# soham2560/MPCHoloNavigation

Measured on AMD Instinct MI355X. Metric: rollouts/sec per computeVelocityCommands() tick, higher is better.
Workload: dtype f32

## Files before the change

mpcholonavigation_amd/csrc/smpc_api.cpp:

```cpp

#include "smpc_ctx.h"

#include <emmintrin.h>

namespace smpc_impl {

thread_local std::string g_create_error;

int fail(smpc_ctx* c, int code, const std::string& msg)
{
  if (c) c->err = msg; else g_create_error = msg;
  return code;
}

int wait_map_upload(smpc_ctx* c)
{
  if (!c->map_pending) return SMPC_OK;
  HIPCK(c, hipEventSynchronize(c->ev_map));
  c->map_pending = false;
  return SMPC_OK;
}

void bar_copy(void* dev_dst, const void* host_src, size_t n)
{
// ... 495 lines not shown
  if (cfg->motion_model > SMPC_MODEL_ACKERMANN)
    return fail(nullptr, SMPC_ERR_UNSUPPORTED, "motion_model must be Omni, DiffDrive or Ackermann");
  if (cfg->motion_model == SMPC_MODEL_ACKERMANN && !(cfg->ackermann_min_turning_r >= 0.f))
    return fail(nullptr, SMPC_ERR_INVALID, "ackermann_min_turning_r must be >= 0");
  if (cfg->time_steps > 64 * SMPC_MAX_R)
    return fail(nullptr, SMPC_ERR_UNSUPPORTED, "time_steps > 256");
  if (!(cfg->temperature > 0.f) || !(cfg->model_dt > 0.f))
    return fail(nullptr, SMPC_ERR_INVALID, "temperature and model_dt must be > 0");
  int ndev = 0;
  hipError_t e = hipGetDeviceCount(&ndev);
  if (e != hipSuccess || ndev == 0)
    return fail(nullptr, SMPC_ERR_DEVICE,
                std::string("no HIP device: ") + (e != hipSuccess ? hipGetErrorString(e) : "count 0") +
                " (libsmpc has no CPU fallback)");
  smpc_ctx* c = new (std::nothrow) smpc_ctx();
  if (!c) return fail(nullptr, SMPC_ERR_NOMEM, "out of host memory");
  c->cfg = *cfg;
  c->knobs = read_knobs();
  smpc_critic_params_default(&c->critics);
  c->holonomic = cfg->motion_model == SMPC_MODEL_OMNI;
  c->acker_r = cfg->motion_model == SMPC_MODEL_ACKERMANN ? cfg->ackermann_min_turning_r : -1.f;
  c->c_vx_max = cfg->vx_max; c->c_vx_min = cfg->vx_min; c->c_vy = cfg->vy_max; c->c_wz = cfg->wz_max;
  int dev = cfg->device;
  if (dev < 0) {
    if (hipGetDevice(&dev) != hipSuccess) dev = 0;
  }
  c->device = dev;
#define CK(call)                                                                        \
  do {                                                                                  \
    hipError_t e__ = (call);                                                            \
    if (e__ != hipSuccess) {                                                            \
      g_create_error = std::string(#call) + ": " + hipGetErrorString(e__);              \
      free_ctx(c);                                                                      \
      return SMPC_ERR_DEVICE;                                                           \
    }                                                                                   \
  } while (0)
  CK(hipSetDevice(dev));
  hipDeviceProp_t prop;
  CK(hipGetDeviceProperties(&prop, dev));
  c->num_cu = prop.multiProcessorCount > 0 ? prop.multiProcessorCount : 256;
  {
    int large_bar = 0;
    if (hipDeviceGetAttribute(&large_bar, hipDeviceAttributeIsLargeBar, dev) != hipSuccess) large_bar = 0;
    c->bar_tick = large_bar != 0 && c->knobs.bar_tick;
    if (c->bar_tick && c->knobs.hdp_flush) {
      c->hdp_flush = find_hdp_flush(dev);
      if (!c->hdp_flush) c->bar_tick = false;
    }
  }
  CK(hipStreamCreateWithFlags(&c->own_stream, hipStreamNonBlocking));
  c->stream = c->own_stream;
  if (getenv("SMPC_LANE_TIMELINE")) {
    static_assert(SMPC_TAIL_STAMPS_AT == 8192 + kMaxGrid * 8, "the tail's stamps sit behind the lane pass's");
    CK(hipMalloc(&c->d_timeline, (8192 + kMaxGrid * 8 + 8 * 16) * sizeof(unsigned long long)));
    CK(hipMemset(c->d_timeline, 0, (8192 + kMaxGrid * 8 + 8 * 16) * sizeof(unsigned long long)));
  }
  CK(hipEventCreate(&c->ev0));
  CK(hipEventCreateWithFlags(&c->ev_map, hipEventDisableTiming));
  CK(hipEventCreate(&c->ev1));
  for (auto& e : c->evp) CK(hipEventCreate(&e));
  const uint32_t T = cfg->time_steps;
  c->R = T <= 64 ? 1 : (T <= 128 ? 2 : 4);
  const size_t n = static_cast<size_t>(cfg->batch_size) * T * sizeof(float);
  CK(hipMalloc(&c->d_nvx, n));
  CK(hipMalloc(&c->d_nvy, n));
  if (!c->holonomic) CK(hipMemset(c->d_nvy, 0, n));
  CK(hipMalloc(&c->d_nwz, n));
  {
    bool tpr = cfg->batch_size >= kLaneMinBatch && cfg->time_steps <= kLaneMaxT;
    if (cfg->time_steps <= 64 && cfg->time_steps >= 36 && (cfg->time_steps & 3u) == 0 && cfg->batch_size >= kSplitMinBatch &&
        !c->knobs.no_split)
      tpr = true;
    if (cfg->flags & SMPC_FLAG_WAVE_PER_ROLLOUT) tpr = false;
    if (cfg->flags & SMPC_FLAG_LANE_PER_ROLLOUT) {
      tpr = true;
      c->lane_forced = true;
    }
    if (c->knobs.pass == Knobs::kWave) tpr = false;
    if (c->knobs.pass == Knobs::kLane || c->knobs.pass == Knobs::kSplit) {
      tpr = true;
      c->lane_forced = true;
    }
    if (cfg->flags & SMPC_FLAG_STORE_TRAJECTORIES) tpr = false;
    const size_t ngm = static_cast<size_t>(SMPC_GM_ROLLOUTS(cfg->batch_size)) * T * sizeof(float);
    if (3ull * ngm >= (1ull << 32)) tpr = false;
    c->use_tpr = tpr;
    if (tpr) {
      CK(hipMalloc(&c->d_tvx, 3 * ngm));
      c->d_tvy = c->d_tvx + ngm / sizeof(float);
      c->d_twz = c->d_tvy + ngm / sizeof(float);
      if (!c->holonomic) CK(hipMemset(c->d_tvy, 0, ngm));
      CK(lane_set_lds_limit(static_cast<int>(kLdsPerCu)));
      CK(split_set_lds_limit(static_cast<int>(kLdsPerCu)));
    }
  }
  CK(hipMalloc(&c->d_costs[0], cfg->batch_size * sizeof(float)));
  CK(hipMalloc(&c->d_costs[1], cfg->batch_size * sizeof(float)));
  CK(hipMemset(c->d_costs[0], 0, cfg->batch_size * sizeof(float)));
  CK(hipMemset(c->d_costs[1], 0, cfg->batch_size * sizeof(float)));
  if (cfg->flags & SMPC_FLAG_STORE_TRAJECTORIES) {
    for (int i = 0; i < 3; ++i) {
      CK(hipMalloc(&c->d_traj[i], n));
      CK(hipMemset(c->d_traj[i], 0, n));
    }
  }
  c->tick_cap = tick_layout(T, SMPC_MAX_PATH).total;
  CK(hipMalloc(&c->d_tick, c->tick_cap));
  CK(hipHostMalloc(&c->h_tick, c->tick_cap, hipHostMallocDefault));
// ... 526 lines not shown
  return SMPC_OK;
}

int smpc_set_stream(smpc_ctx* c, void* hip_stream)
{
  if (!c) return SMPC_ERR_INVALID;
  const int rc = wait_map_upload(c);
  if (rc != SMPC_OK) return rc;
  c->stream = hip_stream == SMPC_STREAM_OWN ? c->own_stream : static_cast<hipStream_t>(hip_stream);
  return SMPC_OK;
}

int smpc_debug_tail_timeline(smpc_ctx* c, unsigned long long* out)
{
  if (!c || !out || !c->d_timeline) return SMPC_ERR_INVALID;
  HIPCK(c, hipSetDevice(c->device));
  HIPCK(c, hipStreamSynchronize(c->stream));
  HIPCK(c, hipMemcpy(out, c->d_timeline + SMPC_TAIL_STAMPS_AT, 8 * 16 * sizeof(unsigned long long), hipMemcpyDeviceToHost));
  return SMPC_OK;
}

int smpc_debug_lane_timeline(smpc_ctx* c, double* out, uint32_t* n_blocks)
{
  if (!c || !out || !c->d_timeline) return SMPC_ERR_INVALID;
  HIPCK(c, hipSetDevice(c->device));
  HIPCK(c, hipStreamSynchronize(c->stream));
  const uint32_t nb = c->plan.lane.grid;
  std::vector<unsigned long long> h(static_cast<size_t>(nb) * 8);
  HIPCK(c, hipMemcpy(h.data(), c->d_timeline, h.size() * sizeof(h[0]), hipMemcpyDeviceToHost));
  unsigned long long t0 = ~0ull;
  for (uint32_t b = 0; b < nb; ++b) t0 = std::min(t0, h[b * 8]);
  for (int k = 0; k < 7; ++k) {
    std::vector<double> v;
    for (uint32_t b = 0; b < nb; ++b)
      if (h[b * 8 + k]) v.push_back(static_cast<double>(h[b * 8 + k] - (k ? h[b * 8 + k - 1] : t0)));
    std::sort(v.begin(), v.end());
    out[3 * k] = v.empty() ? 0 : v.front();
    out[3 * k + 1] = v.empty() ? 0 : v[v.size() / 2];
    out[3 * k + 2] = v.empty() ? 0 : v.back();
  }
  std::vector<unsigned long long> hw(static_cast<size_t>(nb) * 8);
  HIPCK(c, hipMemcpy(hw.data(), c->d_timeline + 8192, hw.size() * sizeof(hw[0]), hipMemcpyDeviceToHost));
  for (int w = 0; w < 8; ++w) {
    std::vector<double> v;
    for (uint32_t b = 0; b < nb; ++b)
      if (hw[b * 8 + w] && h[b * 8 + 2]) v.push_back(static_cast<double>(hw[b * 8 + w] - h[b * 8 + 2]));
    std::sort(v.begin(), v.end());
    out[21 + w] = v.empty() ? 0 : v[v.size() / 2];
  }
  if (n_blocks) *n_blocks = nb;
  return SMPC_OK;
}

const char* smpc_debug_last_pass_kernel(void) {return smpc_last_pass_kernel;}

int smpc_debug_bar_tick(const smpc_ctx* c) {return c && c->bar_tick ? 1 : 0;}

int smpc_set_profile(smpc_ctx* c, int enable)
{
  if (!c) return SMPC_ERR_INVALID;
  if (enable) c->cfg.flags |= SMPC_FLAG_PROFILE;
  else c->cfg.flags &= ~static_cast<uint32_t>(SMPC_FLAG_PROFILE);
  return SMPC_OK;
}
}
```

mpcholonavigation_amd/csrc/smpc_dev.h:

```cpp
#ifndef SMPC_DEV_H_
#define SMPC_DEV_H_

#include <stdint.h>

#define SD_OBSTACLES 0x001u
#define SD_PATH_ALIGN 0x002u
#define SD_PATH_FOLLOW 0x004u
#define SD_GOAL_ANGLE 0x008u
#define SD_PREFER_FORWARD 0x010u
#define SD_USE_PATH_YAW 0x020u
#define SD_ACCUMULATE 0x040u
#define SD_STORE_TRAJ 0x080u
#define SD_TRACK_UNKNOWN 0x100u
#define SD_NEED_FURTHEST 0x200u
#define SD_LOCAL_FURTHEST 0x400u
#define SD_CONSTRAINT 0x800u
#define SD_COST 0x1000u
#define SD_GOAL 0x2000u
#define SD_TWIRLING 0x4000u
#define SD_PATH_ANGLE 0x8000u
#define SD_DEADBAND 0x10000u
#define SD_FP_OBSTACLES 0x20000u
#define SD_FP_COST 0x40000u
#define SD_PATH_ALIGN_LEGACY 0x80000u
// ... 74 lines not shown
  float ga_weight, ga_goal_yaw;
  uint32_t ga_power;
  float pfw_weight;
  uint32_t pfw_power;
  float con_weight, con_max_vel, con_min_vel;
  uint32_t con_power;
  float con_acker_r;
  const float* lut_cost;
  float cost_w254, cost_collision_cost;
  float cost_critical;
  uint32_t cost_near_goal;
  uint32_t cost_power;
  double goal_x, goal_y;
  float goal_weight;
  uint32_t goal_power;
  float tw_weight;
  uint32_t tw_power;
  const uint8_t* pang_active;
  float pang_weight;
  uint32_t pang_power, pang_offset;
  int32_t pang_correct;
  const uint8_t* pal_active;
  float pal_weight, pal_eval;
  uint32_t pal_power;
  double db_vx, db_vy, db_wz;
  float db_weight;
  uint32_t db_power;
  uint32_t fp_n;
  float fp_pic;
  const SmpcLut* lut_fp;
  double fp_x[16], fp_y[16];
  float g_vx, g_vy, g_wz;
  float neg_inv_temp;
  float k2;
  float* partials;
  uint32_t* furthest_out;
  uint32_t tail;
  uint32_t* tail_counter;
  float* tuple;
  SmpcFinal fin;
  unsigned long long* timeline;
  uint32_t canary_echo;
  uint32_t tick_inline;
  uint32_t u_inline;
  uint16_t io_px, io_py, io_pyaw, io_D, io_pf_idx, io_pvalid, io_pa_active, io_pang_active, io_pal_active, io_pad;
  uint8_t tick_bytes[1536] __attribute__((aligned(16)));
  float u_arg[3 * 64] __attribute__((aligned(16)));
};
#define SMPC_INLINE_TICK_CAP 1536u
#define SMPC_MAX_GRID 2048u
#define SMPC_CANARY_SLOT(T) (SMPC_MAX_GRID * (4u + 3u * (T)))
#define SMPC_TAIL_MAX_GRID 512u
#define SMPC_TAIL_STAMPS_AT (8192u + 2048u * 8u)
static inline uint32_t smpc_tail_lds_bytes(uint32_t T) {return (512u + 64u + ((4u + 3u * T + 63u) / 64u) * 2048u + 4u) * 4u;}

#if defined(__HIPCC__)
struct SmpcTickPtrs {
  const float* u;
  const float* px;
  const float* py;
  const float* pyaw;
  const float* D;
  const uint32_t* pf_idx;
  const uint8_t* pvalid;
  const uint8_t* pa_active;
  const uint8_t* pang_active;
  const uint8_t* pal_active;
};
__device__ __forceinline__ SmpcTickPtrs smpc_tick_ptrs(const SmpcDev& p, bool kernarg_is_dev)
{
  SmpcTickPtrs t{p.u, p.px, p.py, p.pyaw, p.D, p.pf_idx, p.pvalid, p.pa_active, p.pang_active, p.pal_active};
#if defined(__HIP_DEVICE_COMPILE__)
  if (kernarg_is_dev && p.tick_inline) {
    const uint8_t* k = reinterpret_cast<const uint8_t*>(__builtin_amdgcn_kernarg_segment_ptr()) +
                       __builtin_offsetof(SmpcDev, tick_bytes);
    if (p.u_inline) t.u = reinterpret_cast<const float*>(reinterpret_cast<const uint8_t*>(__builtin_amdgcn_kernarg_segment_ptr()) +
                                                         __builtin_offsetof(SmpcDev, u_arg));
    t.px = reinterpret_cast<const float*>(k + p.io_px);
    t.py = reinterpret_cast<const float*>(k + p.io_py);
    t.pyaw = reinterpret_cast<const float*>(k + p.io_pyaw);
    t.D = reinterpret_cast<const float*>(k + p.io_D);
    t.pf_idx = reinterpret_cast<const uint32_t*>(k + p.io_pf_idx);
    t.pvalid = k + p.io_pvalid;
    t.pa_active = k + p.io_pa_active;
    t.pang_active = k + p.io_pang_active;
    t.pal_active = k + p.io_pal_active;
  }
#else
  (void)kernarg_is_dev;
#endif
  return t;
}
#endif

#if defined(__HIPCC__)
__host__ __device__
#endif
static inline uint32_t smpc_furthest_index(float F) {return (uint32_t)(F + 0.5f);}


#define SMPC_P2P_MAX_RANKS 16
struct SmpcP2P {
  float* peer[SMPC_P2P_MAX_RANKS];
  uint32_t world, rank;
  uint32_t slot_floats;
  uint32_t xseq;
// ... 28 lines not shown
```

mpcholonavigation_amd/csrc/smpc_lane.hip:

```cpp

#include <hip/hip_runtime.h>
#include <stdint.h>
#include <stdio.h>

#include <type_traits>

#include "smpc_dev.h"
#include "smpc_device_math.h"
#include "smpc_tail.h"
#include "smpc_lane_common.h"
#include "smpc_inst.h"

#ifndef WAVE
#define WAVE 64
#endif
#ifndef LANE_X_RR_NOLOAD
#define LANE_X_RR_NOLOAD 0
#endif
#define LANE_BLOCK 512
#ifndef LANE_BLOCK_RR
#define LANE_BLOCK_RR 512
#endif

#ifndef LANE_X_GAMMA_N
#define LANE_X_GAMMA_N 0
#endif
#ifndef LANE_X_GAMMA_UC
#define LANE_X_GAMMA_UC 1
#endif
#ifndef LANE_X_FURTHEST_WINDOW
#define LANE_X_FURTHEST_WINDOW 1
#endif
#ifndef LANE_X_PFW_MIN
#define LANE_X_PFW_MIN 1
#endif
#ifndef LANE_X_CELL_AX
#define LANE_X_CELL_AX 1
#endif
#ifndef LANE_X_PIN_LDS
#define LANE_X_PIN_LDS 0
#endif
#ifndef LANE_X_PARK_STEP
#define LANE_X_PARK_STEP 0
#endif
#ifndef LANE_X_CONST_VGPR
#define LANE_X_CONST_VGPR 0
#endif

#ifndef LANE_X_PFW_BARE
#define LANE_X_PFW_BARE 1
#endif
#ifndef LANE_X_NOISE_QUAD
#define LANE_X_NOISE_QUAD 1
#endif
#ifndef LANE_X_PRIO_ITER
#define LANE_X_PRIO_ITER 1
#endif

template <bool TO_GM>
__global__ void __launch_bounds__(256) smpc_relayout(const float* __restrict__ src, float* __restrict__ dst,
                                                    uint32_t B, uint32_t T)
{
  __shared__ float tile[32][33];
  const uint32_t b0 = blockIdx.x * 32, t0 = blockIdx.y * 32;
  const uint32_t lx = threadIdx.x & 31, ly = threadIdx.x >> 5;
  if (TO_GM) {
    for (uint32_t k = ly; k < 32; k += 8) {
      const uint32_t b = b0 + k, t = t0 + lx;
      tile[k][lx] = (b < B && t < T) ? src[(size_t)b * T + t] : 0.f;
    }
    __syncthreads();
    for (uint32_t k = ly; k < 32; k += 8) {
      const uint32_t t = t0 + k, b = b0 + lx;
      if (b < B && t < T) dst[SMPC_GM_INDEX(b, t, T)] = tile[lx][k];
    }
  } else {
    for (uint32_t k = ly; k < 32; k += 8) {
      const uint32_t t = t0 + k, b = b0 + lx;
      tile[lx][k] = (b < B && t < T) ? src[SMPC_GM_INDEX(b, t, T)] : 0.f;
    }
    __syncthreads();
    for (uint32_t k = ly; k < 32; k += 8) {
      const uint32_t b = b0 + k, t = t0 + lx;
      if (b < B && t < T) dst[(size_t)b * T + t] = tile[k][lx];
    }
  }
}

hipError_t smpc_launch_relayout(const float* src, float* dst, uint32_t B, uint32_t T, bool to_gm, hipStream_t st)
{
  const dim3 grid((B + 31) / 32, (T + 31) / 32);
  if (to_gm) hipLaunchKernelGGL(smpc_relayout<true>, grid, dim3(256), 0, st, src, dst, B, T);
  else hipLaunchKernelGGL(smpc_relayout<false>, grid, dim3(256), 0, st, src, dst, B, T);
  return hipGetLastError();
}

__global__ void __launch_bounds__(64) smpc_lane_reduce_kernel(const float* __restrict__ v,
                                                              const float* __restrict__ w,
                                                              float* __restrict__ out)
{
  const int lane = threadIdx.x;
  float V[64];
#pragma unroll
  for (int t = 0; t < 64; ++t) V[t] = v[lane * 64 + t];
  const LaneW lw = lane_weights(w[lane], lane);
  out[lane] = lane_reduce64(V, lw, lane);
}

hipError_t smpc_launch_lane_reduce(const float* v, const float* w, float* out, hipStream_t st)
// ... 114 lines not shown
```

mpcholonavigation_amd/csrc/smpc_lane_common.h:

```cpp
#ifndef SMPC_LANE_COMMON_H_
#define SMPC_LANE_COMMON_H_

#include <hip/hip_runtime.h>
#include <stdint.h>

#include "smpc_dev.h"
#include "smpc_device_math.h"

#ifndef WAVE
#define WAVE 64
#endif

typedef unsigned u32x2 __attribute__((ext_vector_type(2)));
typedef const float __attribute__((address_space(4))) * cfloat_p;
typedef float f32x32 __attribute__((ext_vector_type(32)));
typedef float f32x4 __attribute__((ext_vector_type(4)));
typedef float f32x2 __attribute__((ext_vector_type(2)));
#define LANE_PARK_STRIDE 68

struct LaneW {
  float wa, wb;
};

#define SMPC_DPP_NODE(NAME, CTRL, BANKS)                                                    \
// ... 13 lines not shown
template <int CTRL>
__device__ __forceinline__ float dpp_mov(float v)
{
  return __uint_as_float(
    (uint32_t)__builtin_amdgcn_update_dpp(0, (int)__float_as_uint(v), CTRL, 0xF, 0xF, false));
}

template <int K, int Rr>
__device__ __forceinline__ float lane_reduce_node(const float (&V)[64], const LaneW& w, int lane)
{
  if constexpr (K == 0) {
    return V[Rr];
  } else {
    const float a = lane_reduce_node<K - 1, Rr>(V, w, lane);
    const float b = lane_reduce_node<K - 1, Rr + (64 >> K)>(V, w, lane);
    if constexpr (K == 1) {
      const u32x2 s = __builtin_amdgcn_permlane32_swap(__float_as_uint(a), __float_as_uint(b),
                                                       false, false);
      return fmaf(w.wa, __uint_as_float(s.x), w.wb * __uint_as_float(s.y));
    } else if constexpr (K == 2) {
      const u32x2 s = __builtin_amdgcn_permlane16_swap(__float_as_uint(a), __float_as_uint(b),
                                                       false, false);
      return __uint_as_float(s.x) + __uint_as_float(s.y);
    } else if constexpr (K == 3) {
      return node_bit3(a, b);
    } else if constexpr (K == 4) {
      return node_bit2(a, b);
    } else if constexpr (K == 5) {
      const float ta = a + dpp_mov<0x4E>(a);
      const float tb = b + dpp_mov<0x4E>(b);
      return (lane & 2) ? tb : ta;
    } else {
      const float ta = a + dpp_mov<0xB1>(a);
      const float tb = b + dpp_mov<0xB1>(b);
      return (lane & 1) ? tb : ta;
    }
  }
}

__device__ __forceinline__ LaneW lane_weights(float w, int lane)
{
  const float wo = __shfl_xor(w, 32, WAVE);
  LaneW r;
  r.wa = lane < 32 ? w : wo;
  r.wb = lane < 32 ? wo : w;
  return r;
}

__device__ __forceinline__ float lane_reduce64(const float (&V)[64], const LaneW& w, int lane)
{
  return lane_reduce_node<6, 0>(V, w, lane);
}

__device__ __forceinline__ int cvt_floor_i32(float q)
{
  int r;
  asm("v_cvt_flr_i32_f32 %0, %1" : "=v"(r) : "v"(q));
  return r;
}

__device__ __forceinline__ float add_min_zero(float acc, float x)
{
  float m;
  asm("v_min_f32 %1, 0, %2\n\tv_add_f32 %0, %0, %1" : "+v"(acc), "=&v"(m) : "v"(x));
  return acc;
}

__device__ __forceinline__ uint32_t cell_byte_exact(const SmpcDev& p, uint8_t* s_map, float x,
                                                    float y, uint32_t slot)
{
  const uint32_t nwin = (uint32_t)(p.win_w * p.win_h);
  uint32_t mx = 0, my = 0;
  bool on = cell_index_exact((double)x, p.ox, p.res, p.W, mx);
  on = cell_index_exact((double)y, p.oy, p.res, p.H, my) && on;
  if (!on) return nwin;
  const uint32_t wx = mx - (uint32_t)p.win_x0, wy = my - (uint32_t)p.win_y0;
  if (wx < (uint32_t)p.win_w && wy < (uint32_t)p.win_h) return wy * p.win_w + wx;
  s_map[nwin + 1 + slot] = p.map[(size_t)my * p.W + mx];
  return nwin + 1 + slot;
}

#endif
```

mpcholonavigation_amd/csrc/smpc_lane_pass.inc:

```
template <bool FULL, bool OBST, bool MANY, int NCH, bool RR, bool GA = false, bool QUADS = FULL, int TC = 0, bool DEP = false>
__global__ void __launch_bounds__(RR ? LANE_BLOCK_RR : LANE_BLOCK, (RR && LANE_BLOCK_RR == 256) ? 3 : 1)
LANE_PASS_KERNEL(const SmpcDev p0, const SmpcLds L, const SmpcDev* __restrict__ many)
{
  constexpr bool POW = LANE_PASS_POW;
  static_assert(RR || NCH == 1, "parked controls: one chunk of 64 steps");
  static_assert(!POW || (!MANY && !RR && !DEP), "cost powers: the single-context parking form of the five critics");
  static_assert(!FULL || QUADS, "T == 64 is a multiple of four");
  static_assert(TC == 0 || (!FULL && QUADS && !RR && TC < 64 && (TC & 3) == 0), "compile-time horizon: whole quads below 64");
  static_assert(!DEP || (OBST && !RR && !GA), "deployed-list instances: parking form");
  const SmpcDev& p = MANY ? many[blockIdx.y] : p0;
  const SmpcTickPtrs tk{p.u, p.px, p.py, p.pyaw, p.D, p.pf_idx, p.pvalid, p.pa_active, p.pang_active, p.pal_active};
  extern __shared__ __attribute__((aligned(16))) unsigned char smem[];
  uint8_t* s_map = smem;
  const SmpcLut* s_lut = reinterpret_cast<const SmpcLut*>(smem + L.off_lut);
  float* s_px = reinterpret_cast<float*>(smem + L.off_px);
  float* s_py = reinterpret_cast<float*>(smem + L.off_py);
  float* s_D = reinterpret_cast<float*>(smem + L.off_D) + 1;
  f32x4* s_pts4 = reinterpret_cast<f32x4*>(smem + L.off_pts4);
  float* s_su2 = reinterpret_cast<float*>(smem + L.off_scr) - 4;

  constexpr int BLK = RR ? LANE_BLOCK_RR : LANE_BLOCK;
  const int blk = blockDim.x;
  const int tid = threadIdx.x;
  const int lane = tid & (WAVE - 1);
// ... 82 lines not shown
      s_py[i] = qy;
      if (seg) s_D[i] = tk.D[i];
      s_pts4[i] = f32x4{qx, qy, (seg && tk.pvalid[i]) ? 1.0f : 0.f, 0.f};
    }
  }
  __syncthreads();
  stamp(1);

  const cfloat_p cu = (cfloat_p)(uintptr_t)p.u;
  const uint32_t T = FULL ? 64u * NCH : (TC ? (uint32_t)TC : p.T), B = p.B;
  const uint32_t noise_bytes = T * SMPC_GM_ROLLOUTS(B) * 4u;
  const __amdgpu_buffer_rsrc_t rn = __builtin_amdgcn_make_buffer_rsrc(const_cast<float*>(p.tvx), 0, 3u * noise_bytes, 0x00020000);
  const float dt = p.dt, yaw0 = p.yaw0;
  const double x0 = p.x0, y0 = p.y0;
  uint32_t S = 0;
  if (p.flags & SD_NEED_FURTHEST) {
    S = p.d_furthest ? smpc_furthest_index(*p.d_furthest) : p.furthest_hint;
    if (S >= p.P) S = p.P ? p.P - 1 : 0;
  }
  if (lane == 0) {
    s_D[-1] = -3.0e38f;
    s_D[S] = 3.0e38f;
  }
  const bool pa_on = (p.flags & SD_PATH_ALIGN) && p.P > 0 && tk.pa_active[S] && S > 0;
  float pf_x = 0.f, pf_y = 0.f;
  if ((p.flags & SD_PATH_FOLLOW) && p.P > 0) {
    const uint32_t idx = tk.pf_idx[S];
    pf_x = tk.px[idx];
    pf_y = tk.py[idx];
  }
  const uint32_t bs_iters = S > 1 ? 32u - (uint32_t)__builtin_clz(S - 1) : 0u;
  float pa_inv_spacing = 0.f;
  if (pa_on && S > 1 && tk.D[S - 1] > 0.f) pa_inv_spacing = (float)(S - 1) / tk.D[S - 1];
  const bool want_local_furthest = (p.flags & SD_NEED_FURTHEST) && (p.flags & SD_LOCAL_FURTHEST);
  const bool con_on = DEP && (p.flags & SD_CONSTRAINT) != 0, tw_on = DEP && (p.flags & SD_TWIRLING) != 0;
  const float k_con = p.dt * p.con_weight, k_tw = p.tw_weight / (float)(FULL ? 64 * NCH : (TC ? TC : (int)p.T));
  const bool cost_mode = DEP && (p.flags & SD_COST) != 0;
  constexpr bool ga_on = GA;
  const uint32_t nquad = (T + 3u) >> 2;

  float m_run = 3.0e38f, s_run = 0.f;
  float Ux[NCH], Uy[NCH], Uz[NCH];
#pragma unroll
  for (int h = 0; h < NCH; ++h) Ux[h] = Uy[h] = Uz[h] = 0.f;
  float F_local = 0.f;
  uint32_t n_noncoll = 0;

  const uint32_t ngroups = (B + WAVE - 1) / WAVE;
  const uint32_t gw = blockIdx.x * nwave + wave;
  const uint32_t nW = gridDim.x * nwave;

  using T_ = std::true_type;
  using F_ = std::false_type;
  auto group_body = [&](auto safe_c, const uint32_t grp) -> bool {
    constexpr bool SAFE = decltype(safe_c)::value;
    const uint32_t b = grp * WAVE + lane;
    const bool live = b < B;
    const uint32_t bl = live ? b : B - 1;
    f32x32 PX0, PX1, PY0, PY1;
    if (!FULL && !RR) PX0 = PX1 = PY0 = PY1 = (f32x32)(0.f);

    float cpx = p.svx, cpy = p.svy, cpz = p.swz;
    float acc_yaw = 0.f, ax = 0.f, ay = 0.f;
    float cs_prev = p.cos0, sn_prev = p.sin0;
    float x = 0.f, y = 0.f;
    float crit = 0.f, rep = 0.f;
    float yaw_max = 0.f;
    float alive = 1.0f;
    uint32_t cell_q = 256u;
    f32x2 e_q = {0.f, 0.f};
    [[maybe_unused]] const uint32_t lds_lut = (uint32_t)(uintptr_t)s_lut, lds_map = (uint32_t)(uintptr_t)s_map;
    auto lookup_wait = [&]() {
#if LANE_X_PIN_LDS
      asm volatile("s_waitcnt lgkmcnt(0)" : "+v"(cell_q), "+v"(e_q));
#endif
    };
    auto lookup_accumulate = [&]() {
      alive = e_q.x < 0.f ? 0.f : alive;
      crit = fmaf(alive, e_q.x, crit);
      rep = fmaf(alive, e_q.y, rep);
    };
#if LANE_X_PIN_LDS
    auto lookup_issue_entry = [&]() {
      const uint32_t a = lds_lut + (cell_q << 3);
      asm volatile("ds_read_b64 %0, %1" : "=v"(e_q) : "v"(a));
    };
    auto lookup_issue_byte = [&](uint32_t idx) {
      const uint32_t a = lds_map + idx;
      asm volatile("ds_read_u8 %0, %1" : "=v"(cell_q) : "v"(a));
    };
#else
    auto lookup_issue_entry = [&]() {
      const SmpcLut e = s_lut[cell_q];
      e_q = f32x2{e.crit, e.rep};
    };
    auto lookup_issue_byte = [&](uint32_t idx) {cell_q = s_map[idx];};
#endif
    float pfw = 0.f, gx = 0.f, gy = 0.f, gz = 0.f;
    float ga_sum = 0.f;
    float ext = 0.f;
    float traj_dist = 0.f, pa_sum = 0.f, pa_num = 0.f, sx_prev = p.x00f, sy_prev = p.y00f;
    uint32_t path_pt = 0;

#if LANE_X_CONST_VGPR
    const float k_rinv = in_vgpr(p.rinvf), k_cx = in_vgpr(p.cxf), k_cy = in_vgpr(p.cyf);
#else
// ... 285 lines not shown
          }
#endif
        };
        uint32_t q = 0;
        for (; q + 1 < qh; q += 2) {
          quad_lo(q);
          quad_lo(q + 1);
        }
        if (q < qh) quad_lo(q);
        q = 8;
        for (; q + 1 < nquad; q += 2) {
          quad_hi(q);
          quad_hi(q + 1);
        }
        if (q < nquad) quad_hi(q);
      } else {
#pragma unroll 2
        for (uint32_t q = 0; q < qh; ++q) {
          float cq[12];
          run_quad(F_{}, T_{}, q, cq);
#if !LANE_X_PARK_STEP
#pragma unroll
          for (int i = 0; i < 4; ++i) {
            PX0[8 * i + q] = cq[3 * i];
            PY0[8 * i + q] = cq[3 * i + 1];
            park[(4 * q + i) * LANE_PARK_STRIDE + lane] = cq[3 * i + 2];
          }
#endif
        }
#pragma unroll 2
        for (uint32_t q = 8; q < nquad; ++q) {
          float cq[12];
          run_quad(T_{}, T_{}, q, cq);
#if !LANE_X_PARK_STEP
#pragma unroll
          for (int i = 0; i < 4; ++i) {
            PX1[8 * i + (q - 8)] = cq[3 * i];
            PY1[8 * i + (q - 8)] = cq[3 * i + 1];
            park[(4 * q + i) * LANE_PARK_STRIDE + lane] = cq[3 * i + 2];
          }
#endif
        }
      }
    }
    if (OBST) {
      lookup_wait();
      lookup_accumulate();
      lookup_issue_entry();
      lookup_wait();
      lookup_accumulate();
    }
    if (!SAFE && __builtin_expect(__any(!(yaw_max < 65536.0f) || !(fabsf(acc_yaw) < 65536.0f)), 0)) return true;

    x = (float)(x0 + (double)ax);
    y = (float)(y0 + (double)ay);

    if (want_local_furthest) {
      auto block_d2 = [&](const float* bx, const float* by, float (&dd)[4]) {
        const f32x4 qx = *reinterpret_cast<const f32x4*>(bx);
        const f32x4 qy = *reinterpret_cast<const f32x4*>(by);
#pragma unroll
        for (int e = 0; e < 4; ++e) {
          const float ex = qx[e] - x, ey = qy[e] - y;
          dd[e] = ex * ex + ey * ey;
        }
      };
      float best = 3.4028234663852886e38f;
      uint32_t bj = 0;
      const uint32_t P4 = (p.P + 3u) & ~3u;
      constexpr bool kWindow = LANE_X_FURTHEST_WINDOW && !GA && !DEP && !MANY;
      const uint32_t j_lo = (kWindow && (S >> 2) > 3u) ? ((S >> 2) - 3u) << 2 : 0u;
      for (uint32_t j = j_lo; j < P4; j += 4) {
        float dd[4];
        block_d2(s_px + j, s_py + j, dd);
        const float mn = fminf(fminf(dd[0], dd[1]), fminf(dd[2], dd[3]));
        if (mn < best) {
          best = mn;
          bj = j;
        }
      }
      auto point_F = [&]() -> float {
        float dd[4];
        block_d2(s_px + bj, s_py + bj, dd);
        const uint32_t bi = bj + (dd[0] == best ? 0u : dd[1] == best ? 1u : dd[2] == best ? 2u : dd[3] == best ? 3u : 0u);
        float F = (float)bi;
        if (bi + 1 < p.P) {
          const float nx = s_px[bi + 1], ny = s_py[bi + 1];
          const float sgx = nx - s_px[bi], sgy = ny - s_py[bi];
          const float d_next = (nx - x) * (nx - x) + (ny - y) * (ny - y);
          const float seg2 = sgx * sgx + sgy * sgy;
          const float tt = seg2 > 0.f ? 0.5f + 0.5f * (best - d_next) * fast_rcp(seg2) : 0.f;
          F = fmaxf(F + fminf(fmaxf(tt, -0.45f), 0.45f), 0.f);
        }
        return F;
      };
      float F = point_F();
      float m = live ? F : 0.f;
      for (int o = 32; o > 0; o >>= 1) m = fmaxf(m, __shfl_xor(m, o, WAVE));
      if (kWindow && j_lo) {
        const unsigned long long holders = __ballot(live && F == m);
        bool below = false;
        if (holders) {
          const int wl = __builtin_ctzll(holders);
          const float wx = __shfl(x, wl, WAVE), wy = __shfl(y, wl, WAVE), wbest = __shfl(best, wl, WAVE);
          for (uint32_t k = (uint32_t)lane; k < j_lo; k += WAVE) {
            const float ex = s_px[k] - wx, ey = s_py[k] - wy;
            below = below || (ex * ex + ey * ey <= wbest);
          }
        }
        if (__builtin_expect(__any(below), 0)) {
          for (uint32_t jj = j_lo; jj > 0; jj -= 4) {
            const uint32_t j = jj - 4;
            float dd[4];
            block_d2(s_px + j, s_py + j, dd);
            const float mn = fminf(fminf(dd[0], dd[1]), fminf(dd[2], dd[3]));
            if (mn <= best) {
              best = mn;
              bj = j;
            }
          }
          F = point_F();
          m = live ? F : 0.f;
          for (int o = 32; o > 0; o >>= 1) m = fmaxf(m, __shfl_xor(m, o, WAVE));
        }
      }
      F_local = fmaxf(F_local, m);
    }
    float cost = (p.flags & SD_ACCUMULATE) ? p.costs_prev[bl] : 0.f;
    if constexpr (POW) {
      if (OBST) {
        const bool collided = alive == 0.f;
        const float raw = collided ? p.obs_collision_cost : crit;
        const float v = (p.obs_critical_w * raw) + (p.obs_repulsion_w * rep / (float)T);
        cost = add_cost_pow(cost, (double)v, p.obs_power);
        n_noncoll += (uint32_t)__popcll(__ballot(live && !collided));
      }
      if (pa_on) {
        const float c_pa = pa_num > 0.f ? pa_sum / pa_num : 0.f;
        cost = add_cost_pow(cost, (double)(c_pa * p.pa_weight), p.pa_power);
      }
      if (p.flags & SD_PATH_FOLLOW) {
        const double ddx = (double)(x - pf_x), ddy = (double)(y - pf_y);
        cost = add_cost_pow(cost, (double)in_vgpr(p.pf_weight) * sqrt_unscaled(ddx * ddx + ddy * ddy), p.pf_power);
      }
      if (ga_on) {
        const double Td = (FULL || TC) ? (double)T : (double)in_vgpr((float)T);
        cost = add_cost_pow(cost, (double)ga_sum / Td * (double)in_vgpr(p.ga_weight), p.ga_power);
      }
#if LANE_X_PFW_MIN
      if (p.flags & SD_PREFER_FORWARD) cost = add_cost_pow(cost, (double)((pfw * -dt) * p.pfw_weight), p.pfw_power);
#else
      if (p.flags & SD_PREFER_FORWARD) cost = add_cost_pow(cost, (double)(pfw * p.pfw_weight), p.pfw_power);
#endif
#if LANE_X_GAMMA_UC
      cost += p.g_vx * (gx - s_su2[0]);
      cost += p.g_wz * (gz - s_su2[2]);
      cost += p.g_vy * (gy - s_su2[1]);
#else
      cost += p.g_vx * gx;
      cost += p.g_wz * gz;
      cost += p.g_vy * gy;
#endif
    } else {
      float lin = 0.f, uni = 0.f;
      if (OBST) {
        const bool collided = alive == 0.f;
        if (cost_mode) {
          const float k = p.cost_w254 / (float)T;
          lin = collided ? 0.f : k * rep;
          uni = collided ? k * p.cost_collision_cost : 0.f;
        } else {
          lin = (collided ? 0.f : p.obs_critical_w * crit) + p.obs_rep_over_T * rep;
          uni = collided ? p.obs_critical_w * p.obs_collision_cost : 0.f;
        }
        n_noncoll += (uint32_t)__popcll(__ballot(live && !collided));
      }
      if constexpr (DEP) lin += ext;
      if (p.flags & SD_PATH_FOLLOW) {
        const float fdx = x - pf_x, fdy = y - pf_y;
        uni += p.pf_weight * fast_sqrt(fdx * fdx + fdy * fdy);
      }
#if LANE_X_PFW_MIN
      if (p.flags & SD_PREFER_FORWARD) lin += (pfw * -dt) * p.pfw_weight;
#else
      if (p.flags & SD_PREFER_FORWARD) lin += pfw * p.pfw_weight;
#endif
      if (ga_on) uni += (ga_sum / (float)T) * p.ga_weight;
#if LANE_X_GAMMA_UC
      lin += p.g_vx * (gx - s_su2[0]);
      lin += p.g_wz * (gz - s_su2[2]);
      lin += p.g_vy * (gy - s_su2[1]);
#else
      lin += p.g_vx * gx;
      lin += p.g_wz * gz;
      lin += p.g_vy * gy;
#endif
      cost += uni + lin;
      if (pa_on) {
        const float c_pa = pa_num > 0.f ? pa_sum * fast_rcp(pa_num) : 0.f;
        cost += c_pa * p.pa_weight;
      }
    }
    if (live) p.costs[b] = cost;

    float cmin = live ? cost : 3.0e38f;
    for (int o = 32; o > 0; o >>= 1) cmin = fminf(cmin, __shfl_xor(cmin, o, WAVE));
    const float m_new = fminf(m_run, cmin);
    const float f = __builtin_amdgcn_exp2f(p.k2 * (m_run - m_new));
    const float w = live ? __builtin_amdgcn_exp2f(p.k2 * (cost - m_new)) : 0.f;
    float wsum = w;
    for (int o = 32; o > 0; o >>= 1) wsum += __shfl_xor(wsum, o, WAVE);
    s_run = fmaf(s_run, f, wsum);
    m_run = m_new;

    const LaneW lw = lane_weights(w, lane);
    if constexpr (RR) {
#pragma unroll
      for (int h = 0; h < NCH; ++h) {
#pragma unroll
        for (int ctrl = 0; ctrl < 3; ++ctrl) {
          float V[64];
#pragma unroll
          for (int t = 0; t < 64; ++t) V[t] = LANE_X_RR_NOLOAD ? (float)t : ld(ctrl, 64u * h + t);
          __builtin_amdgcn_sched_barrier(0);
#pragma unroll
          for (int t = 0; t < 64; ++t) {
            const uint32_t tt = 64u * h + t;
            const float c = ldu(ctrl, tt) + V[t];
            V[t] = (FULL || tt < T) ? c : 0.f;
          }
          const float r = lane_reduce64(V, lw, lane);
          if (ctrl == 0) Ux[h] = fmaf(Ux[h], f, r);
          else if (ctrl == 1) Uy[h] = fmaf(Uy[h], f, r);
          else Uz[h] = fmaf(Uz[h], f, r);
        }
      }
    } else {
      {
        float V[64];
#pragma unroll
        for (int t = 0; t < 32; ++t) {
          V[t] = PX0[8 * (t & 3) + (t >> 2)];
          V[32 + t] = PX1[8 * (t & 3) + (t >> 2)];
        }
        Ux[0] = fmaf(Ux[0], f, lane_reduce64(V, lw, lane));
#pragma unroll
        for (int t = 0; t < 32; ++t) {
          V[t] = PY0[8 * (t & 3) + (t >> 2)];
          V[32 + t] = PY1[8 * (t & 3) + (t >> 2)];
        }
        Uy[0] = fmaf(Uy[0], f, lane_reduce64(V, lw, lane));
      }
      {
        s_w[lane] = w;
        __builtin_amdgcn_fence(__ATOMIC_RELEASE, "wavefront");
        __builtin_amdgcn_wave_barrier();
        __builtin_amdgcn_fence(__ATOMIC_ACQUIRE, "wavefront");
        const f32x4* row = reinterpret_cast<const f32x4*>(park + lane * LANE_PARK_STRIDE);
        float acc0 = 0.f, acc1 = 0.f;
#pragma unroll
        for (int bq = 0; bq < 16; bq += 2) {
          const f32x4 w0 = reinterpret_cast<const f32x4*>(s_w)[bq], c0 = row[bq];
          const f32x4 w1 = reinterpret_cast<const f32x4*>(s_w)[bq + 1], c1 = row[bq + 1];
#pragma unroll
          for (int e = 0; e < 4; ++e) {
            acc0 = fmaf(w0[e], c0[e], acc0);
            acc1 = fmaf(w1[e], c1[e], acc1);
          }
        }
        Uz[0] = fmaf(Uz[0], f, acc0 + acc1);
        __builtin_amdgcn_wave_barrier();
      }
    }
    return false;
  };

  stamp(2);
  int stamp_k = 3;
  for (uint32_t grp = gw; grp < ngroups; grp += nW) {
    if (__builtin_expect(group_body(F_{}, grp), 0)) group_body(T_{}, grp);
    if (stamp_k < 5) stamp(stamp_k++);
  }

  if (__builtin_expect(p.timeline != nullptr, 0) && lane == 0)
    p.timeline[8192 + blockIdx.x * 8 + wave] = __builtin_amdgcn_s_memtime();
  __syncthreads();
  stamp(5);
  const uint32_t TL = 4 + 3 * T;
  float* myp = reinterpret_cast<float*>(smem + L.off_scr) + (size_t)wave * L.scr_stride;
  if (lane == 0) {
    myp[0] = m_run;
    myp[1] = s_run;
    myp[2] = F_local;
    myp[3] = (float)n_noncoll;
  }
#pragma unroll
  for (int h = 0; h < NCH; ++h) {
    const uint32_t tt = 64u * h + (uint32_t)lane;
    if (tt < T) {
      myp[4 + tt] = Ux[h];
      myp[4 + T + tt] = Uy[h];
      myp[4 + 2 * T + tt] = Uz[h];
    }
  }
  __syncthreads();
  const float* allp = reinterpret_cast<const float*>(smem + L.off_scr);
  float bm = 3.0e38f;
  for (int w = 0; w < nwave; ++w) bm = fminf(bm, allp[(size_t)w * L.scr_stride]);
  float* outp = p.partials + (size_t)blockIdx.x * TL;
  for (uint32_t i = tid; i < TL; i += blockDim.x) {
    float acc = 0.f;
    if (i == 0) {
      acc = bm;
    } else if (i == 2) {
      for (int w = 0; w < nwave; ++w) acc = fmaxf(acc, allp[(size_t)w * L.scr_stride + 2]);
    } else if (i == 3) {
      for (int w = 0; w < nwave; ++w) acc += allp[(size_t)w * L.scr_stride + 3];
    } else {
      for (int w = 0; w < nwave; ++w) {
        const float mw = allp[(size_t)w * L.scr_stride];
        const float sc = __builtin_amdgcn_exp2f(p.k2 * (mw - bm));
        acc += sc * allp[(size_t)w * L.scr_stride + i];
      }
    }
    smpc_store_partial(outp + i, acc);
  }
  stamp(6);
  if (!(p.flags & SD_ACCUMULATE) && blockIdx.x == 0 && tid == 0) outp[SMPC_CANARY_SLOT(T)] = cu[-4];
  if constexpr (!MANY && !RR) {
    if (p.tail) smpc_grid_tail<(RR ? LANE_BLOCK_RR : LANE_BLOCK) / 64>(p, smem);
  }
// ... 2 lines not shown
```

Baseline: 5.483 billion.

## Pair the x/y lane reductions and interleave the LDS weight walk in the epilogue

The per-group epilogue now reduces the x and y control sums together through a paired DPP/permlane reduction tree, and splits the LDS dot-product walk for the yaw channel into two halves. The LDS loads are issued between the reduction halves so their latency overlaps with the cross-lane shuffles. The furthest-point max reduction is also folded into the cost-min shuffle loop so both travel together, with readlane replacing shfl for the winner broadcast. It adds inline asm DPP sequences and more live registers (two 64-float arrays plus the load buffers), which risks register pressure and lower occupancy. Optional loop-end timeline stamps and a debug readout are added as well.

New measurement: 5.481 billion, median of 3. No clear change (-0.0%).

```diff
diff --git a/mpcholonavigation_amd/csrc/smpc_api.cpp b/mpcholonavigation_amd/csrc/smpc_api.cpp
--- a/mpcholonavigation_amd/csrc/smpc_api.cpp
+++ b/mpcholonavigation_amd/csrc/smpc_api.cpp
@@ -571,8 +571,9 @@
   c->stream = c->own_stream;
   if (getenv("SMPC_LANE_TIMELINE")) {
     static_assert(SMPC_TAIL_STAMPS_AT == 8192 + kMaxGrid * 8, "the tail's stamps sit behind the lane pass's");
-    CK(hipMalloc(&c->d_timeline, (8192 + kMaxGrid * 8 + 8 * 16) * sizeof(unsigned long long)));
-    CK(hipMemset(c->d_timeline, 0, (8192 + kMaxGrid * 8 + 8 * 16) * sizeof(unsigned long long)));
+    static_assert(SMPC_LANE_LOOP_STAMPS_AT == SMPC_TAIL_STAMPS_AT + 8 * 16, "the loop-end stamps sit behind the tail's");
+    CK(hipMalloc(&c->d_timeline, (SMPC_LANE_LOOP_STAMPS_AT + kMaxGrid * 2) * sizeof(unsigned long long)));
+    CK(hipMemset(c->d_timeline, 0, (SMPC_LANE_LOOP_STAMPS_AT + kMaxGrid * 2) * sizeof(unsigned long long)));
   }
   CK(hipEventCreate(&c->ev0));
   CK(hipEventCreateWithFlags(&c->ev_map, hipEventDisableTiming));
@@ -1205,6 +1206,36 @@
   return SMPC_OK;
 }
 
+int smpc_debug_lane_timeline_split(smpc_ctx* c, double* out)
+{
+  if (!c || !out || !c->d_timeline) return SMPC_ERR_INVALID;
+  HIPCK(c, hipSetDevice(c->device));
+  HIPCK(c, hipStreamSynchronize(c->stream));
+  const uint32_t nb = c->plan.lane.grid;
+  std::vector<unsigned long long> h(static_cast<size_t>(nb) * 8), hl(static_cast<size_t>(nb) * 2);
+  HIPCK(c, hipMemcpy(h.data(), c->d_timeline, h.size() * sizeof(h[0]), hipMemcpyDeviceToHost));
+  HIPCK(c, hipMemcpy(hl.data(), c->d_timeline + SMPC_LANE_LOOP_STAMPS_AT, hl.size() * sizeof(hl[0]), hipMemcpyDeviceToHost));
+  for (int g = 0; g < 2; ++g) {
+    std::vector<double> loop, epi;
+    for (uint32_t b = 0; b < nb; ++b) {
+      const unsigned long long t0 = h[b * 8 + 2 + g], tl = hl[b * 2 + g], t1 = h[b * 8 + 3 + g];
+      if (!t0 || !tl || !t1) continue;
+      loop.push_back(static_cast<double>(tl - t0));
+      epi.push_back(static_cast<double>(t1 - tl));
+    }
+    std::sort(loop.begin(), loop.end());
+    std::sort(epi.begin(), epi.end());
+    double* o = out + 6 * g;
+    o[0] = loop.empty() ? 0 : loop.front();
+    o[1] = loop.empty() ? 0 : loop[loop.size() / 2];
+    o[2] = loop.empty() ? 0 : loop.back();
+    o[3] = epi.empty() ? 0 : epi.front();
+    o[4] = epi.empty() ? 0 : epi[epi.size() / 2];
+    o[5] = epi.empty() ? 0 : epi.back();
+  }
+  return SMPC_OK;
+}
+
 const char* smpc_debug_last_pass_kernel(void) {return smpc_last_pass_kernel;}
 
 int smpc_debug_bar_tick(const smpc_ctx* c) {return c && c->bar_tick ? 1 : 0;}
diff --git a/mpcholonavigation_amd/csrc/smpc_dev.h b/mpcholonavigation_amd/csrc/smpc_dev.h
--- a/mpcholonavigation_amd/csrc/smpc_dev.h
+++ b/mpcholonavigation_amd/csrc/smpc_dev.h
@@ -150,6 +150,7 @@
 #define SMPC_CANARY_SLOT(T) (SMPC_MAX_GRID * (4u + 3u * (T)))
 #define SMPC_TAIL_MAX_GRID 512u
 #define SMPC_TAIL_STAMPS_AT (8192u + 2048u * 8u)
+#define SMPC_LANE_LOOP_STAMPS_AT (SMPC_TAIL_STAMPS_AT + 8u * 16u)
 static inline uint32_t smpc_tail_lds_bytes(uint32_t T) {return (512u + 64u + ((4u + 3u * T + 63u) / 64u) * 2048u + 4u) * 4u;}
 
 #if defined(__HIPCC__)
diff --git a/mpcholonavigation_amd/csrc/smpc_lane.hip b/mpcholonavigation_amd/csrc/smpc_lane.hip
--- a/mpcholonavigation_amd/csrc/smpc_lane.hip
+++ b/mpcholonavigation_amd/csrc/smpc_lane.hip
@@ -55,6 +55,15 @@
 #endif
 #ifndef LANE_X_PRIO_ITER
 #define LANE_X_PRIO_ITER 1
+#endif
+#ifndef LANE_X_EPI_PAIR
+#define LANE_X_EPI_PAIR 1
+#endif
+#ifndef LANE_X_EPI_FENCE
+#define LANE_X_EPI_FENCE 0
+#endif
+#ifndef LANE_X_EPI_MINMAX
+#define LANE_X_EPI_MINMAX 1
 #endif
 
 template <bool TO_GM>
diff --git a/mpcholonavigation_amd/csrc/smpc_lane_common.h b/mpcholonavigation_amd/csrc/smpc_lane_common.h
--- a/mpcholonavigation_amd/csrc/smpc_lane_common.h
+++ b/mpcholonavigation_amd/csrc/smpc_lane_common.h
@@ -89,6 +89,78 @@
   return lane_reduce_node<6, 0>(V, w, lane);
 }
 
+struct LanePair {
+  float x, y;
+};
+
+#define SMPC_DPP_NODE2(NAME, CTRL, BANKS)                                                   \
+  __device__ __forceinline__ LanePair NAME(float ax, float bx, float ay, float by)          \
+  {                                                                                         \
+    LanePair t;                                                                             \
+    asm("s_nop 1\n\t"                                                                       \
+        "v_add_f32_dpp %0, %2, %2 " CTRL " row_mask:0xf bank_mask:0xf\n\t"                  \
+        "v_add_f32_dpp %1, %4, %4 " CTRL " row_mask:0xf bank_mask:0xf\n\t"                  \
+        "v_add_f32_dpp %0, %3, %3 " CTRL " row_mask:0xf bank_mask:" BANKS "\n\t"            \
+        "v_add_f32_dpp %1, %5, %5 " CTRL " row_mask:0xf bank_mask:" BANKS                   \
+        : "=&v"(t.x), "=&v"(t.y)                                                            \
+        : "v"(ax), "v"(bx), "v"(ay), "v"(by));                                              \
+    return t;                                                                               \
+  }
+SMPC_DPP_NODE2(node2_bit3, "row_ror:8", "0xc")
+SMPC_DPP_NODE2(node2_bit2, "row_half_mirror", "0xa")
+
+template <int K>
+__device__ __forceinline__ LanePair lane_reduce_join2(const LanePair a, const LanePair b, const LaneW& w, int lane)
+{
+  static_assert(K >= 1 && K <= 6, "one of the six levels");
+  if constexpr (K == 1) {
+    const u32x2 sx = __builtin_amdgcn_permlane32_swap(__float_as_uint(a.x), __float_as_uint(b.x), false, false);
+    const u32x2 sy = __builtin_amdgcn_permlane32_swap(__float_as_uint(a.y), __float_as_uint(b.y), false, false);
+    const float mx = w.wb * __uint_as_float(sx.y), my = w.wb * __uint_as_float(sy.y);
+    return LanePair{fmaf(w.wa, __uint_as_float(sx.x), mx), fmaf(w.wa, __uint_as_float(sy.x), my)};
+  } else if constexpr (K == 2) {
+    const u32x2 sx = __builtin_amdgcn_permlane16_swap(__float_as_uint(a.x), __float_as_uint(b.x), false, false);
+    const u32x2 sy = __builtin_amdgcn_permlane16_swap(__float_as_uint(a.y), __float_as_uint(b.y), false, false);
+    return LanePair{__uint_as_float(sx.x) + __uint_as_float(sx.y), __uint_as_float(sy.x) + __uint_as_float(sy.y)};
+  } else if constexpr (K == 3) {
+    return node2_bit3(a.x, b.x, a.y, b.y);
+  } else if constexpr (K == 4) {
+    return node2_bit2(a.x, b.x, a.y, b.y);
+  } else if constexpr (K == 5) {
+    const float tax = a.x + dpp_mov<0x4E>(a.x), tay = a.y + dpp_mov<0x4E>(a.y);
+    const float tbx = b.x + dpp_mov<0x4E>(b.x), tby = b.y + dpp_mov<0x4E>(b.y);
+    return LanePair{(lane & 2) ? tbx : tax, (lane & 2) ? tby : tay};
+  } else {
+    const float tax = a.x + dpp_mov<0xB1>(a.x), tay = a.y + dpp_mov<0xB1>(a.y);
+    const float tbx = b.x + dpp_mov<0xB1>(b.x), tby = b.y + dpp_mov<0xB1>(b.y);
+    return LanePair{(lane & 1) ? tbx : tax, (lane & 1) ? tby : tay};
+  }
+}
+
+template <int K, int Rr>
+__device__ __forceinline__ LanePair lane_reduce_node2(const float (&VX)[64], const float (&VY)[64], const LaneW& w, int lane)
+{
+  if constexpr (K == 0) {
+    return LanePair{VX[Rr], VY[Rr]};
+  } else {
+    const LanePair a = lane_reduce_node2<K - 1, Rr>(VX, VY, w, lane);
+    const LanePair b = lane_reduce_node2<K - 1, Rr + (64 >> K)>(VX, VY, w, lane);
+    return lane_reduce_join2<K>(a, b, w, lane);
+  }
+}
+
+template <int Rr>
+__device__ __forceinline__ LanePair lane_reduce_half2(const float (&VX)[64], const float (&VY)[64], const LaneW& w, int lane)
+{
+  static_assert(Rr == 0 || Rr == 1, "the two subtrees below the last level");
+  return lane_reduce_node2<5, Rr>(VX, VY, w, lane);
+}
+
+__device__ __forceinline__ LanePair lane_reduce_top2(const LanePair lo, const LanePair hi, const LaneW& w, int lane)
+{
+  return lane_reduce_join2<6>(lo, hi, w, lane);
+}
+
 __device__ __forceinline__ int cvt_floor_i32(float q)
 {
   int r;
diff --git a/mpcholonavigation_amd/csrc/smpc_lane_pass.inc b/mpcholonavigation_amd/csrc/smpc_lane_pass.inc
--- a/mpcholonavigation_amd/csrc/smpc_lane_pass.inc
+++ b/mpcholonavigation_amd/csrc/smpc_lane_pass.inc
@@ -158,6 +158,7 @@
 
   using T_ = std::true_type;
   using F_ = std::false_type;
+  int stamp_k = 3;
   auto group_body = [&](auto safe_c, const uint32_t grp) -> bool {
     constexpr bool SAFE = decltype(safe_c)::value;
     const uint32_t b = grp * WAVE + lane;
@@ -549,57 +550,51 @@
     }
     if (!SAFE && __builtin_expect(__any(!(yaw_max < 65536.0f) || !(fabsf(acc_yaw) < 65536.0f)), 0)) return true;
 
+    if (__builtin_expect(p.timeline != nullptr, 0) && tid == 0 && stamp_k < 5)
+      p.timeline[SMPC_LANE_LOOP_STAMPS_AT + blockIdx.x * 2 + (stamp_k - 3)] = __builtin_amdgcn_s_memtime();
+
     x = (float)(x0 + (double)ax);
     y = (float)(y0 + (double)ay);
 
-    if (want_local_furthest) {
-      auto block_d2 = [&](const float* bx, const float* by, float (&dd)[4]) {
-        const f32x4 qx = *reinterpret_cast<const f32x4*>(bx);
-        const f32x4 qy = *reinterpret_cast<const f32x4*>(by);
-#pragma unroll
-        for (int e = 0; e < 4; ++e) {
-          const float ex = qx[e] - x, ey = qy[e] - y;
-          dd[e] = ex * ex + ey * ey;
-        }
-      };
-      float best = 3.4028234663852886e38f;
-      uint32_t bj = 0;
-      const uint32_t P4 = (p.P + 3u) & ~3u;
-      constexpr bool kWindow = LANE_X_FURTHEST_WINDOW && !GA && !DEP && !MANY;
-      const uint32_t j_lo = (kWindow && (S >> 2) > 3u) ? ((S >> 2) - 3u) << 2 : 0u;
-      for (uint32_t j = j_lo; j < P4; j += 4) {
-        float dd[4];
-        block_d2(s_px + j, s_py + j, dd);
-        const float mn = fminf(fminf(dd[0], dd[1]), fminf(dd[2], dd[3]));
-        if (mn < best) {
-          best = mn;
-          bj = j;
-        }
-      }
-      auto point_F = [&]() -> float {
-        float dd[4];
-        block_d2(s_px + bj, s_py + bj, dd);
-        const uint32_t bi = bj + (dd[0] == best ? 0u : dd[1] == best ? 1u : dd[2] == best ? 2u : dd[3] == best ? 3u : 0u);
-        float F = (float)bi;
-        if (bi + 1 < p.P) {
-          const float nx = s_px[bi + 1], ny = s_py[bi + 1];
-          const float sgx = nx - s_px[bi], sgy = ny - s_py[bi];
-          const float d_next = (nx - x) * (nx - x) + (ny - y) * (ny - y);
-          const float seg2 = sgx * sgx + sgy * sgy;
-          const float tt = seg2 > 0.f ? 0.5f + 0.5f * (best - d_next) * fast_rcp(seg2) : 0.f;
-          F = fmaxf(F + fminf(fmaxf(tt, -0.45f), 0.45f), 0.f);
-        }
-        return F;
-      };
-      float F = point_F();
-      float m = live ? F : 0.f;
-      for (int o = 32; o > 0; o >>= 1) m = fmaxf(m, __shfl_xor(m, o, WAVE));
+    constexpr bool kMinMax = LANE_X_EPI_MINMAX && !RR && !GA && !DEP && !MANY && !POW;
+    constexpr bool kWindow = LANE_X_FURTHEST_WINDOW && !GA && !DEP && !MANY;
+    float F = 0.f, m = 0.f, best = 3.4028234663852886e38f;
+    uint32_t bj = 0, j_lo = 0;
+    auto block_d2 = [&](const float* bx, const float* by, float (&dd)[4]) {
+      const f32x4 qx = *reinterpret_cast<const f32x4*>(bx);
+      const f32x4 qy = *reinterpret_cast<const f32x4*>(by);
+#pragma unroll
+      for (int e = 0; e < 4; ++e) {
+        const float ex = qx[e] - x, ey = qy[e] - y;
+        dd[e] = ex * ex + ey * ey;
+      }
+    };
+    auto point_F = [&]() -> float {
+      float dd[4];
+      block_d2(s_px + bj, s_py + bj, dd);
+      const uint32_t bi = bj + (dd[0] == best ? 0u : dd[1] == best ? 1u : dd[2] == best ? 2u : dd[3] == best ? 3u : 0u);
+      float Fp = (float)bi;
+      if (bi + 1 < p.P) {
+        const float nx = s_px[bi + 1], ny = s_py[bi + 1];
+        const float sgx = nx - s_px[bi], sgy = ny - s_py[bi];
+        const float d_next = (nx - x) * (nx - x) + (ny - y) * (ny - y);
+        const float seg2 = sgx * sgx + sgy * sgy;
+        const float tt = seg2 > 0.f ? 0.5f + 0.5f * (best - d_next) * fast_rcp(seg2) : 0.f;
+        Fp = fmaxf(Fp + fminf(fmaxf(tt, -0.45f), 0.45f), 0.f);
+      }
+      return Fp;
+    };
+    auto furthest_check = [&]() {
       if (kWindow && j_lo) {
         const unsigned long long holders = __ballot(live && F == m);
         bool below = false;
         if (holders) {
           const int wl = __builtin_ctzll(holders);
-          const float wx = __shfl(x, wl, WAVE), wy = __shfl(y, wl, WAVE), wbest = __shfl(best, wl, WAVE);
+          auto from_lane = [&](float v) -> float {
+            if constexpr (kMinMax) return __int_as_float(__builtin_amdgcn_readlane(__float_as_int(v), wl));
+            else return __shfl(v, wl, WAVE);
+          };
+          const float wx = from_lane(x), wy = from_lane(y), wbest = from_lane(best);
           for (uint32_t k = (uint32_t)lane; k < j_lo; k += WAVE) {
             const float ex = s_px[k] - wx, ey = s_py[k] - wy;
             below = below || (ex * ex + ey * ey <= wbest);
@@ -622,6 +617,25 @@
         }
       }
       F_local = fmaxf(F_local, m);
+    };
+    if (want_local_furthest) {
+      const uint32_t P4 = (p.P + 3u) & ~3u;
+      j_lo = (kWindow && (S >> 2) > 3u) ? ((S >> 2) - 3u) << 2 : 0u;
+      for (uint32_t j = j_lo; j < P4; j += 4) {
+        float dd[4];
+        block_d2(s_px + j, s_py + j, dd);
+        const float mn = fminf(fminf(dd[0], dd[1]), fminf(dd[2], dd[3]));
+        if (mn < best) {
+          best = mn;
+          bj = j;
+        }
+      }
+      F = point_F();
+      if constexpr (!kMinMax) {
+        m = live ? F : 0.f;
+        for (int o = 32; o > 0; o >>= 1) m = fmaxf(m, __shfl_xor(m, o, WAVE));
+        furthest_check();
+      }
     }
     float cost = (p.flags & SD_ACCUMULATE) ? p.costs_prev[bl] : 0.f;
     if constexpr (POW) {
@@ -701,13 +715,27 @@
     if (live) p.costs[b] = cost;
 
     float cmin = live ? cost : 3.0e38f;
-    for (int o = 32; o > 0; o >>= 1) cmin = fminf(cmin, __shfl_xor(cmin, o, WAVE));
+    if constexpr (kMinMax) {
+      m = live ? F : 0.f;
+#pragma unroll
+      for (int o = 32; o > 0; o >>= 1) {
+        const float co = __shfl_xor(cmin, o, WAVE), mo = __shfl_xor(m, o, WAVE);
+        cmin = fminf(cmin, co);
+        m = fmaxf(m, mo);
+      }
+      if (want_local_furthest) furthest_check();
+    } else {
+      for (int o = 32; o > 0; o >>= 1) cmin = fminf(cmin, __shfl_xor(cmin, o, WAVE));
+    }
     const float m_new = fminf(m_run, cmin);
     const float f = __builtin_amdgcn_exp2f(p.k2 * (m_run - m_new));
     const float w = live ? __builtin_amdgcn_exp2f(p.k2 * (cost - m_new)) : 0.f;
+    constexpr bool kEpiPair = LANE_X_EPI_PAIR && !RR;
     float wsum = w;
-    for (int o = 32; o > 0; o >>= 1) wsum += __shfl_xor(wsum, o, WAVE);
-    s_run = fmaf(s_run, f, wsum);
+    if constexpr (!kEpiPair) {
+      for (int o = 32; o > 0; o >>= 1) wsum += __shfl_xor(wsum, o, WAVE);
+      s_run = fmaf(s_run, f, wsum);
+    }
     m_run = m_new;
 
     const LaneW lw = lane_weights(w, lane);
@@ -732,6 +760,65 @@
           else Uz[h] = fmaf(Uz[h], f, r);
         }
       }
+    } else if constexpr (kEpiPair) {
+      s_w[lane] = w;
+      __builtin_amdgcn_fence(__ATOMIC_RELEASE, "wavefront");
+      __builtin_amdgcn_wave_barrier();
+      __builtin_amdgcn_fence(__ATOMIC_ACQUIRE, "wavefront");
+      const f32x4* row = reinterpret_cast<const f32x4*>(park + lane * LANE_PARK_STRIDE);
+      const f32x4* wq = reinterpret_cast<const f32x4*>(s_w);
+      float VX[64], VY[64];
+#pragma unroll
+      for (int t = 0; t < 32; ++t) {
+        VX[t] = PX0[8 * (t & 3) + (t >> 2)];
+        VX[32 + t] = PX1[8 * (t & 3) + (t >> 2)];
+        VY[t] = PY0[8 * (t & 3) + (t >> 2)];
+        VY[32 + t] = PY1[8 * (t & 3) + (t >> 2)];
+      }
+      float acc0 = 0.f, acc1 = 0.f;
+      f32x4 wv[8], cv[8];
+      auto walk_issue = [&](int half) __attribute__((always_inline)) {
+#pragma unroll
+        for (int i = 0; i < 8; ++i) {
+          wv[i] = wq[8 * half + i];
+          cv[i] = row[8 * half + i];
+        }
+      };
+      auto walk_consume = [&]() __attribute__((always_inline)) {
+#pragma unroll
+        for (int i = 0; i < 8; i += 2) {
+#pragma unroll
+          for (int e = 0; e < 4; ++e) {
+            acc0 = fmaf(wv[i][e], cv[i][e], acc0);
+            acc1 = fmaf(wv[i + 1][e], cv[i + 1][e], acc1);
+          }
+        }
+      };
+      walk_issue(0);
+#if LANE_X_EPI_FENCE
+      __builtin_amdgcn_sched_barrier(0);
+#endif
+      for (int o = 32; o > 0; o >>= 1) wsum += __shfl_xor(wsum, o, WAVE);
+      s_run = fmaf(s_run, f, wsum);
+      const LanePair r0 = lane_reduce_half2<0>(VX, VY, lw, lane);
+#if LANE_X_EPI_FENCE
+      __builtin_amdgcn_sched_barrier(0);
+#endif
+      walk_consume();
+      walk_issue(1);
+#if LANE_X_EPI_FENCE
+      __builtin_amdgcn_sched_barrier(0);
+#endif
+      const LanePair r1 = lane_reduce_half2<1>(VX, VY, lw, lane);
+      const LanePair r = lane_reduce_top2(r0, r1, lw, lane);
+#if LANE_X_EPI_FENCE
+      __builtin_amdgcn_sched_barrier(0);
+#endif
+      walk_consume();
+      Ux[0] = fmaf(Ux[0], f, r.x);
+      Uy[0] = fmaf(Uy[0], f, r.y);
+      Uz[0] = fmaf(Uz[0], f, acc0 + acc1);
+      __builtin_amdgcn_wave_barrier();
     } else {
       {
         float V[64];
@@ -773,7 +860,6 @@
   };
 
   stamp(2);
-  int stamp_k = 3;
   for (uint32_t grp = gw; grp < ngroups; grp += nW) {
     if (__builtin_expect(group_body(F_{}, grp), 0)) group_body(T_{}, grp);
     if (stamp_k < 5) stamp(stamp_k++);
```
